# sv-goat/LLM-Inference-in-Distributed-Edge-Networks

Measured on AMD Instinct MI355X. Metric: WikiText-2 PPL + inter-stage bytes/token, Qwen2-0.5B 2-stage split; tokens/sec, higher is better.
Workload: dtype fp32; 1 GPU; model=qwen2-0.5b, global_batch=256, seq_len=512, stride=32, parallelism=local-pp2, codec=mixed_int4_int8, importance=regular_importance, transport=local, hip_graphs=True, gemm_precision=h3 split-fp16 (fp32-accurate), last_layer_rows=scored

## Files before the change

csrc/gemm.hip:

```cpp
#include <type_traits>
#include "common.h"
#include <algorithm>
#include <cstdlib>
#include <cstring>

enum { EPI_NONE = 0, EPI_BIAS = 1, EPI_RESID = 2, EPI_BIAS_RESID = 3, EPI_BIAS_GELU = 4, EPI_SWIGLU = 5,
       EPI_QKV_ROPE = 6, EPI_LSE = 7,
       EPI_F32 = 8, EPI_F32_BIAS = 9, EPI_F32_RESID = 10, EPI_F32_BIAS_RESID = 11, EPI_H3_BIAS_GELU = 12,
       EPI_H3_SWIGLU = 13, EPI_F32_QKV_ROPE = 14, EPI_F32_LSE = 15,
       EPI_F32_RESID_CS = 16,
       EPI_H3_LRP_SWIGLU = 17,
       EPI_F32_RESID_NP = 18 };
constexpr bool epi_f32(int e) { return e >= EPI_F32; }
constexpr bool epi_plain(int e) {
  return e == EPI_NONE || e == EPI_BIAS || e == EPI_RESID || e == EPI_BIAS_RESID || e == EPI_F32 ||
         e == EPI_F32_BIAS || e == EPI_F32_RESID || e == EPI_F32_BIAS_RESID || e == EPI_F32_RESID_CS ||
         e == EPI_F32_RESID_NP;
}

struct GemmArgs {
  const bf16_t* A; const bf16_t* B; bf16_t* C;
  int M, N, K, lda, ldb, ldc;
  const bf16_t* bias; const bf16_t* resid; int ldr;
  float* Cf; const float* biasf; const float* residf;
  float* qf; float* kf; float* vtf;
  float* vf;
  f16_t* planes; float* prinv; const float* bnd_a; const float* bnd_b; float bnd_c;
  float np_g, np_rn;
  bf16_t* qout; bf16_t* kout; bf16_t* vtout;
  const float* cosT; const float* sinT;
  int S, Hq, Hkv, s_pad; float q_scale;
  f16_t* kp; f16_t* vp; float kv_sk, kv_sv;
  const int64_t* targets; float* part_max; float* part_sum; float* tgt_logit; int nparts;
  const float* rscale; float* ssq_out;
  const float* colscale;
  const float* ssq_in; int ssq_parts; float norm_inv_k, norm_eps;
  int walk;
  int store_wait = 0;
  int h3k;
  int pairb;
  float alpha = 1.f;
  float out_scale = 1.f;
  float* raw = nullptr;
  bf16_t* rawb = nullptr;
};

__device__ __forceinline__ int a_kcol(const GemmArgs& a, int k) {
  if (a.pairb) return ((k >> 6) & 1 ? 0 : a.h3k) + ((k >> 7) << 6);
  return a.h3k ? h3_acol(k, a.h3k) : k;
}
__device__ __forceinline__ int b_kcol(const GemmArgs& a, int k) { return a.pairb ? (k >> 7) << 6 : k; }

template <bool F16>
__device__ __forceinline__ f32x4_t mfma16x32(bf16x8_t a, bf16x8_t b, f32x4_t c) {
  if constexpr (F16)
    return __builtin_amdgcn_mfma_f32_16x16x32_f16(__builtin_bit_cast(f16x8_t, a), __builtin_bit_cast(f16x8_t, b), c,
                                                  0, 0, 0);
  else
    return __builtin_amdgcn_mfma_f32_16x16x32_bf16(a, b, c, 0, 0, 0);
}

constexpr int BK = 64;
constexpr int GROUP_M = 8;

template <int BM_, int BN_, int NWM_, int NWN_>
struct Cfg {
  static constexpr int BM = BM_, BN = BN_, NWM = NWM_, NWN = NWN_;
  static constexpr int NW = NWM * NWN, NT = 64 * NW;
  static constexpr int WTM = BM / NWM, MI = WTM / 16;
  static_assert(BN / NWN == 64, "wave column slab must be 64");
  static constexpr int A_BYTES = BM * BK * 2, B_BYTES = BN * BK * 2, STAGE = A_BYTES + B_BYTES;
  static constexpr int A_INSTR = BM / 8 / NW, B_INSTR = BN / 8 / NW;
  static constexpr int LDS = 2 * STAGE;
};
using C128 = Cfg<128, 128, 2, 2>;

__device__ __forceinline__ int swz(int r) { return (r >> 1) & 7; }


__device__ __forceinline__ float gelu_erf(float x) { return 0.5f * x * (1.f + erff(x * 0.70710678118654752f)); }
__device__ __forceinline__ float silu(float x) { return fast_silu(x); }

template <int NI, int NW>
__device__ __forceinline__ void stage_ptrs(const bf16_t* __restrict__ src, int ld, int row0, int row_max, int wave,
                                           int lane, const bf16_t* (&p)[NI]) {
#pragma unroll
  for (int i = 0; i < NI; ++i) {
    const int blk = i * NW + wave;
    const int r = blk * 8 + (lane >> 3);
    const int c = (lane & 7) ^ swz(r);
    int gr = row0 + r;
    gr = gr < row_max ? gr : row_max - 1;
    p[i] = src + (size_t)gr * ld + c * 8;
  }
}
template <int NI, int NW>
__device__ __forceinline__ void stage_issue(const bf16_t* const (&p)[NI], int k0, char* lds, int wave) {
#pragma unroll
  for (int i = 0; i < NI; ++i) glds16(p[i] + k0, lds + (i * NW + wave) * 1024);
}

__device__ __forceinline__ bf16x8_t read_frag(const char* lds, int r, int c) {
  return *(const bf16x8_t*)(lds + r * 128 + ((c ^ swz(r)) << 4));
}

__device__ __forceinline__ void swiglu_h3_rowgroup(const GemmArgs& a, const f32x4_t (&acc4)[4], float f, u32x4_t& H,
                                                   u32x4_t& L) {
  const f32x2_t c1 = {-1.4426950408889634f * f, -1.4426950408889634f * f};
  const f32x2_t k2 = {f * f * a.out_scale, f * f * a.out_scale};
  u32x2_t hw[2], lw[2];
#pragma unroll
  for (int p = 0; p < 2; ++p) {
#pragma unroll
    for (int h = 0; h < 2; ++h) {
      const f32x2_t gg = {acc4[2 * p][2 * h], acc4[2 * p][2 * h + 1]};
      const f32x2_t uu = {acc4[2 * p + 1][2 * h], acc4[2 * p + 1][2 * h + 1]};
      f32x2_t o = gg * uu;
      const f32x2_t t = gg * c1;
      f32x2_t e = {__builtin_amdgcn_exp2f(t[0]), __builtin_amdgcn_exp2f(t[1])};
      e = e + f32x2_t{1.f, 1.f};
      o = o * f32x2_t{__builtin_amdgcn_rcpf(e[0]), __builtin_amdgcn_rcpf(e[1])};
      o = o * k2;
      const u32x2_t hl = split2h_pk(o[0], o[1]);
      hw[p][h] = hl[0];
// ... 750 lines not shown
                                            int lane, int wm, int wn) {
  const int g = lane >> 4;
  const int nw = n0 + wn * 112;
  const int P = a.N / 112;
  static_assert(!epi_f32(EPI), "fp32 epilogues of the 224-wide tiles: w4_f32_epilogue_224");
  constexpr bool RES = EPI == EPI_RESID || EPI == EPI_BIAS_RESID;
  u32x2_t rv[w7::MI][w7::NJ];
  float rsv[w7::MI];
#pragma unroll
  for (int i = 0; i < w7::MI; ++i) {
    int mr = m0 + wm * 64 + i * 16 + (lane & 15);
    mr = mr < a.M ? mr : a.M - 1;
    rsv[i] = a.rscale ? a.rscale[mr] : 1.f;
    if constexpr (RES) {
      const bf16_t* rrow = a.resid + (size_t)mr * a.ldr + nw + g * 4;
#pragma unroll
      for (int j = 0; j < w7::NJ; ++j) rv[i][j] = *(const u32x2_t*)(rrow + j * 16);
    }
  }
#pragma unroll
  for (int i = 0; i < w7::MI; ++i) {
    const int m = m0 + wm * 64 + i * 16 + (lane & 15);
    const bool ok = m < a.M;
    const float rs = rsv[i];
    float ss = 0.f;
    u32x2_t w[w7::NJ];
#pragma unroll
    for (int j = 0; j < w7::NJ; ++j) {
      const int n = nw + j * 16 + g * 4;
      float o[4] = {acc[i][j][0] * rs, acc[i][j][1] * rs, acc[i][j][2] * rs, acc[i][j][3] * rs};
      if constexpr (EPI == EPI_BIAS || EPI == EPI_BIAS_RESID) {
        const u32x2_t bw = *(const u32x2_t*)(a.bias + n);
        o[0] += bf_lo(bw[0]); o[1] += bf_hi(bw[0]); o[2] += bf_lo(bw[1]); o[3] += bf_hi(bw[1]);
      }
      if constexpr (RES) {
        const u32x2_t rw = rv[i][j];
        o[0] += bf_lo(rw[0]); o[1] += bf_hi(rw[0]); o[2] += bf_lo(rw[1]); o[3] += bf_hi(rw[1]);
      }
      w[j][0] = pack_bf2(o[0], o[1]);
      w[j][1] = pack_bf2(o[2], o[3]);
      const float v0 = bf_lo(w[j][0]), v1 = bf_hi(w[j][0]), v2 = bf_lo(w[j][1]), v3 = bf_hi(w[j][1]);
      ss += v0 * v0 + v1 * v1 + v2 * v2 + v3 * v3;
    }
    bf16_t* row = a.C + (size_t)(ok ? m : a.M - 1) * a.ldc + nw;
#pragma unroll
    for (int q2 = 0; q2 < 3; ++q2) {
      const u32x4_t wv = pair_swap16(w[2 * q2], w[2 * q2 + 1]);
      if (ok) *(u32x4_t*)(row + q2 * 32 + pair_col(g)) = wv;
    }
    if (ok) *(u32x2_t*)(row + 96 + g * 4) = w[6];
    if (a.ssq_out) {
      ss += __shfl_xor(ss, 16, 64);
      ss += __shfl_xor(ss, 32, 64);
      if (ok && g == 0) a.ssq_out[(size_t)m * P + nw / 112] = ss;
    }
  }
}

namespace w4 {
template <int BN> struct Geo {
  static constexpr int NJ = BN / 32;
  static constexpr int NB = BN / 32;
  static constexpr int BOFF = 32768, TB = 32768 + BN * 128;
  static constexpr int NR = 8 + NJ;
  static constexpr int MF = 8 * NJ;
  static constexpr int LDS = 2 * TB;
  static constexpr int LDS_R3 = 3 * 32768 + 2 * BN * 128;
};
template <int MF, int NR>
__device__ constexpr int slot_pos(int r) { return (r + 1) * MF / NR - 1; }
}

__device__ __forceinline__ int q192_feat(int col) {
  const int q = (col >> 4) & 3;
  return (col & ~63) | ((q == 1 ? 2 : q == 2 ? 1 : q) << 4) | (col & 15);
}

__device__ __forceinline__ void qkv192_bias(const GemmArgs& a, int n0, int lane, int wn, f32x4_t (&bw)[6]) {
  const int nw = n0 + wn * 96;
#pragma unroll
  for (int j = 0; j < 6; ++j) bw[j] = *(const f32x4_t*)(a.biasf + q192_feat(nw + j * 16) + (lane >> 4) * 4);
}

template <int RH>
__device__ __forceinline__ void qkv192_epilogue(const GemmArgs& a, f32x4_t (&c)[4][6], const f32x4_t (&bw)[6], int m0,
                                                int n0, int lane, int vw, int wn) {
  static_assert(RH == 0 || RH == 32, "192-wide QKV tiles: full rotary or none");
  const int g = lane >> 4;
  const int nw = n0 + wn * 96;
  int bi[4], pi[4];
  f32x4_t cs[4][2], sn[4][2];
#pragma unroll
  for (int i = 0; i < 4; ++i) {
    const int m = min(m0 + vw * 64 + i * 16 + (lane & 15), a.M - 1);
    bi[i] = m / a.S;
    pi[i] = m - bi[i] * a.S;
    if constexpr (RH == 32) {
#pragma unroll
      for (int hf = 0; hf < 2; ++hf) {
        cs[i][hf] = *(const f32x4_t*)(a.cosT + pi[i] * 32 + hf * 16 + g * 4);
        sn[i][hf] = *(const f32x4_t*)(a.sinT + pi[i] * 32 + hf * 16 + g * 4);
      }
    }
  }
#pragma unroll
  for (int i = 0; i < 4; ++i) {
    const int m = m0 + vw * 64 + i * 16 + (lane & 15);
    if (m >= a.M) continue;
    const int b = bi[i], pos = pi[i];
#pragma unroll
    for (int p = 0; p < 3; ++p) {
      const int col = nw + 32 * p;
      const int head = col >> 6;
      const int hf = ((col >> 4) & 3) ? 1 : 0;
      const int d = hf * 16 + g * 4;
      f32x4_t lo = c[i][2 * p] * a.alpha + bw[2 * p];
      f32x4_t hi = c[i][2 * p + 1] * a.alpha + bw[2 * p + 1];
      const bool is_v = head >= a.Hq + a.Hkv;
      if (!is_v) {
        if constexpr (RH == 32) {
          const f32x4_t cv = hf ? cs[i][1] : cs[i][0], sv = hf ? sn[i][1] : sn[i][0];
          const f32x4_t l2 = lo * cv - hi * sv;
          hi = hi * cv + lo * sv;
          lo = l2;
        }
        const float sc = head < a.Hq ? a.q_scale : 1.f;
        float* dst = head < a.Hq ? a.qf + (((size_t)b * a.Hq + head) * a.S + pos) * 64
                                 : a.kf + (((size_t)b * a.Hkv + (head - a.Hq)) * a.S + pos) * 64;
        if (head < a.Hq || a.kf) {
          *(f32x4_t*)(dst + d) = lo * sc;
          *(f32x4_t*)(dst + d + 32) = hi * sc;
        }
        if (head >= a.Hq && a.kp) {
          const float l4[4] = {lo[0], lo[1], lo[2], lo[3]}, h4[4] = {hi[0], hi[1], hi[2], hi[3]};
          store_k_planes4(a, b, head - a.Hq, pos, d, l4);
          store_k_planes4(a, b, head - a.Hq, pos, d + 32, h4);
        }
      } else {
        if (a.vf) {
          float* dst = a.vf + (((size_t)b * a.Hkv + (head - a.Hq - a.Hkv)) * a.S + pos) * 64;
          *(f32x4_t*)(dst + d) = lo;
          *(f32x4_t*)(dst + d + 32) = hi;
        }
        if (a.vtf) {
          float* dst = a.vtf + ((size_t)b * a.Hkv + (head - a.Hq - a.Hkv)) * 64 * (size_t)a.s_pad + pos;
#pragma unroll
          for (int r = 0; r < 4; ++r) {
            dst[(size_t)(d + r) * a.s_pad] = lo[r];
            dst[(size_t)(d + 32 + r) * a.s_pad] = hi[r];
          }
        }
        if (a.vp) {
#pragma unroll
          for (int r = 0; r < 4; ++r) {
            store_vt_plane1(a, b, head - a.Hq - a.Hkv, pos, d + r, lo[r]);
            store_vt_plane1(a, b, head - a.Hq - a.Hkv, pos, d + 32 + r, hi[r]);
          }
        }
      }
    }
  }
}

template <int RH>
__device__ __forceinline__ void qkv192_bf16_epilogue(const GemmArgs& a, f32x4_t (&c)[4][6], const float (&rq)[4],
                                                     int m0, int n0, int lane, int vw, int wn) {
  static_assert(RH == 0 || RH == 32, "192-wide QKV tiles: full rotary or none");
  const int g = lane >> 4;
  const int nw = n0 + wn * 96;
  u32x2_t bw[6];
#pragma unroll
  for (int j = 0; j < 6; ++j) bw[j] = *(const u32x2_t*)(a.bias + q192_feat(nw + j * 16) + g * 4);
  int bi[4], pi[4];
  f32x4_t cs[4][2], sn[4][2];
#pragma unroll
  for (int i = 0; i < 4; ++i) {
    const int m = min(m0 + vw * 64 + i * 16 + (lane & 15), a.M - 1);
    bi[i] = m / a.S;
    pi[i] = m - bi[i] * a.S;
    if constexpr (RH == 32) {
#pragma unroll
      for (int hf = 0; hf < 2; ++hf) {
        cs[i][hf] = *(const f32x4_t*)(a.cosT + pi[i] * 32 + hf * 16 + g * 4);
        sn[i][hf] = *(const f32x4_t*)(a.sinT + pi[i] * 32 + hf * 16 + g * 4);
      }
    }
  }
#pragma unroll
  for (int i = 0; i < 4; ++i) {
    const int m = m0 + vw * 64 + i * 16 + (lane & 15);
    if (m >= a.M) continue;
    const int b = bi[i], pos = pi[i];
#pragma unroll
    for (int p = 0; p < 3; ++p) {
      const int col = nw + 32 * p;
      const int head = col >> 6;
      const int hf = ((col >> 4) & 3) ? 1 : 0;
      const int d = hf * 16 + g * 4;
      const u32x2_t bl = bw[2 * p], bh = bw[2 * p + 1];
      f32x4_t lo = c[i][2 * p] * rq[i] + f32x4_t{bf_lo(bl[0]), bf_hi(bl[0]), bf_lo(bl[1]), bf_hi(bl[1])};
      f32x4_t hi = c[i][2 * p + 1] * rq[i] + f32x4_t{bf_lo(bh[0]), bf_hi(bh[0]), bf_lo(bh[1]), bf_hi(bh[1])};
      if (head < a.Hq + a.Hkv) {
        if constexpr (RH == 32) {
          const f32x4_t cv = hf ? cs[i][1] : cs[i][0], sv = hf ? sn[i][1] : sn[i][0];
          const f32x4_t l2 = lo * cv - hi * sv;
          hi = hi * cv + lo * sv;
          lo = l2;
        }
        const float sc = head < a.Hq ? a.q_scale : 1.f;
        bf16_t* dst = head < a.Hq ? a.qout + (((size_t)b * a.Hq + head) * a.S + pos) * 64
                                  : a.kout + (((size_t)b * a.Hkv + (head - a.Hq)) * a.S + pos) * 64;
        *(u32x2_t*)(dst + d) = u32x2_t{pack_bf2(lo[0] * sc, lo[1] * sc), pack_bf2(lo[2] * sc, lo[3] * sc)};
        *(u32x2_t*)(dst + d + 32) = u32x2_t{pack_bf2(hi[0] * sc, hi[1] * sc), pack_bf2(hi[2] * sc, hi[3] * sc)};
      } else {
        bf16_t* dst = a.vtout + ((size_t)b * a.Hkv + (head - a.Hq - a.Hkv)) * 64 * (size_t)a.s_pad + pos;
#pragma unroll
        for (int r = 0; r < 4; ++r) {
          dst[(size_t)(d + r) * a.s_pad] = f2bf(lo[r]);
          dst[(size_t)(d + 32 + r) * a.s_pad] = f2bf(hi[r]);
        }
      }
    }
  }
}

template <int EPI>
__device__ __forceinline__ void w4_f32_epilogue_224(const GemmArgs& a, f32x4_t (&acc)[8][7], int m0, int n0,
                                                    int lane, int wm, int wn) {
  constexpr bool NP = EPI == EPI_F32_RESID_NP;
  constexpr bool RESF = EPI == EPI_F32_RESID || EPI == EPI_F32_BIAS_RESID || EPI == EPI_F32_RESID_CS || NP;
  constexpr bool BIAS = EPI == EPI_F32_BIAS || EPI == EPI_F32_BIAS_RESID;
  constexpr bool CS = EPI == EPI_F32_RESID_CS;
  const int g = lane >> 4;
  const int nw = n0 + wn * 112;
  const int rbase = m0 + wm * 128 + (lane & 15);
  f32x4_t bw[BIAS || CS || NP ? 7 : 1];
  if constexpr (BIAS) {
#pragma unroll
    for (int j = 0; j < 7; ++j) bw[j] = *(const f32x4_t*)(a.biasf + nw + j * 16 + g * 4);
  }
  if constexpr (CS || NP) {
#pragma unroll
// ... 247 lines not shown
      }
    }
  };
  load_rs(m0);
  auto ktile = [&](int t, auto dmab_c, auto end_c) {
    const uint32_t bo = aslot(t), bn = aslot(t + 1);
    const uint32_t boB = PB ? ((t >> 1) & 1) * BSTRIDE : bo, bnB = PB ? (((t + 1) >> 1) & 1) * BSTRIDE : bn;
    __builtin_amdgcn_sched_barrier(0);
    using DM0 = std::integral_constant<int, R3 ? 2 : (SP2 && decltype(dmab_c)::value) ? 4 : 0>;
    if (kt == 0) mma(XA, XB, YA, YB, bo, boB, 1, std::true_type{}, DM0{}, std::true_type{}, dmab_c);
    else mma(XA, XB, YA, YB, bo, boB, 1, std::false_type{}, DM0{}, std::true_type{}, dmab_c);
    __builtin_amdgcn_sched_barrier(0);
    if (t + 1 < total) {
      constexpr int N0 = R3 ? 8 : (SP2 && decltype(dmab_c)::value) ? NB : 0;
      constexpr int TS = epi_tail_stores<EPI, BN>();
      if constexpr (TS > 0 && RING == 0) {
        if (kt == 0 && epi_full) wait_vm_lgkm0<N0 + TS>();
        else wait_vm_lgkm0<N0>();
      } else {
        wait_vm_lgkm0<N0>();
      }
    } else {
      asm volatile("s_waitcnt lgkmcnt(0)" ::: "memory");
    }
    if constexpr ((BN == 256 || BN == 192) && (RING == 0 || (SP2 && !decltype(dmab_c)::value))) {
#pragma unroll
      for (int i = 0; i < 8; ++i) asm volatile("" : "+v"(rs[i]));
    }
    __builtin_amdgcn_s_barrier();
    __builtin_amdgcn_sched_barrier(0);
    mma(YA, YB, XA, XB, bn, bnB, 0, std::false_type{}, std::integral_constant<int, R3 ? 3 : SP2 ? 5 : 1>{},
        std::true_type{}, dmab_c);
    __builtin_amdgcn_sched_barrier(0);
    asm volatile("s_waitcnt lgkmcnt(0)" ::: "memory");
    ++kt;
    if (decltype(end_c)::value && kt == nk) {
      MFMA_DRAIN();
      __builtin_amdgcn_sched_barrier(0);
      if constexpr (BN == 256 && EPI == EPI_H3_SWIGLU) {
        swiglu_h3_lines_4w<8>(a, acc, rs, m0, n0, lane, wm, wn);
        __builtin_amdgcn_sched_barrier(0);
      } else if constexpr (BN == 256 && EPI == EPI_H3_LRP_SWIGLU) {
        lrp_swiglu_4w(a, acc, m0, n0, lane, wm, wn);
        __builtin_amdgcn_sched_barrier(0);
      } else if constexpr (BN == 256) {
#pragma unroll
        for (int qd = 0; qd < 4; ++qd) {
          const int ih = qd >> 1, h = qd & 1;
          f32x4_t c[4][4];
          float rq[4];
#pragma unroll
          for (int i = 0; i < 4; ++i) {
            rq[i] = rs[ih * 4 + i];
#pragma unroll
            for (int j = 0; j < 4; ++j) {
              c[i][j] = acc[ih * 4 + i][h * 4 + j];
              asm volatile("" : "+v"(c[i][j]));
            }
          }
          if (n0 + wn * 128 + h * 64 < a.N) gemm_epilogue<EPI, RH, CQ>(a, c, m0, n0, lane, wm * 2 + ih, wn * 2 + h, rq);
          __builtin_amdgcn_sched_barrier(0);
        }
      } else if constexpr (BN == 192) {
        f32x4_t bw[6];
        if constexpr (EPI != EPI_QKV_ROPE) qkv192_bias(a, n0, lane, wn, bw);
#pragma unroll
        for (int ih = 0; ih < 2; ++ih) {
          f32x4_t c[4][6];
#pragma unroll
          for (int i = 0; i < 4; ++i)
#pragma unroll
            for (int j = 0; j < 6; ++j) {
              c[i][j] = acc[ih * 4 + i][j];
              asm volatile("" : "+v"(c[i][j]));
            }
          if constexpr (EPI == EPI_QKV_ROPE) {
            const float rq[4] = {rs[ih * 4], rs[ih * 4 + 1], rs[ih * 4 + 2], rs[ih * 4 + 3]};
            qkv192_bf16_epilogue<RH>(a, c, rq, m0, n0, lane, wm * 2 + ih, wn);
          } else {
            qkv192_epilogue<RH>(a, c, bw, m0, n0, lane, wm * 2 + ih, wn);
          }
          __builtin_amdgcn_sched_barrier(0);
        }
      } else if constexpr (epi_f32(EPI)) {
        w4_f32_epilogue_224<EPI>(a, acc, m0, n0, lane, wm, wn);
        __builtin_amdgcn_sched_barrier(0);
      } else {
#pragma unroll
        for (int ih = 0; ih < 2; ++ih) {
          f32x4_t c[4][NJ];
#pragma unroll
          for (int i = 0; i < 4; ++i)
#pragma unroll
            for (int j = 0; j < NJ; ++j) {
              c[i][j] = acc[ih * 4 + i][j];
              asm volatile("" : "+v"(c[i][j]));
            }
          w7_epilogue<EPI>(a, c, m0, n0, lane, wm * 2 + ih, wn);
          __builtin_amdgcn_sched_barrier(0);
        }
      }
      epi_full = a.store_wait && m0 + 256 <= a.M && n0 + BN <= a.N;
      tile += G;
      kt = 0;
      if (tile < walk.end) {
        tile_origin(tile, a.M, a.N, 256, BN, m0, n0);
        load_rs(m0);
      }
#pragma unroll
      for (int i = 0; i < 8; ++i) DS_READ_B128(XA[i], abase[0] + bn, i * 2048);
#pragma unroll
      for (int j = 0; j < NJ; ++j) DS_READ_B128(XB[j], bbase[0] + bnB, j * 2048);
      asm volatile("s_waitcnt lgkmcnt(0)" ::: "memory");
      __builtin_amdgcn_sched_barrier(0);
    }
  };
#pragma unroll 1
  for (int t = 0; t < total; t += PB ? 2 : 1) {
    if constexpr (PB) {
      ktile(t, std::true_type{}, std::false_type{});
      ktile(t + 1, std::false_type{}, std::true_type{});
    } else {
      ktile(t, std::true_type{}, std::true_type{});
    }
  }
  asm volatile("s_waitcnt vmcnt(0)" ::: "memory");
}

static int g_tile_override = 0;

static int num_cus() {
  static int n = 0;
  if (!n) {
    int dev = 0;
    (void)hipGetDevice(&dev);
    if (hipDeviceGetAttribute(&n, hipDeviceAttributeMultiprocessorCount, dev) != hipSuccess || n <= 0) n = 256;
  }
  return n;
}

template <int EPI, int RH, class CF>
static int launch_cfg(const GemmArgs& a, hipStream_t st) {
  const int grid = ((a.M + CF::BM - 1) / CF::BM) * ((a.N + CF::BN - 1) / CF::BN);
  static bool attr = false;
  if (!attr) {
    (void)hipFuncSetAttribute((const void*)gemm_bf16_kernel<EPI, RH, CF>, hipFuncAttributeMaxDynamicSharedMemorySize,
                              CF::LDS);
    attr = true;
  }
  hipLaunchKernelGGL((gemm_bf16_kernel<EPI, RH, CF>), dim3(grid), dim3(CF::NT), CF::LDS, st, a);
  return (int)hipGetLastError();
}

static int g_walk_override = [] {
  const char* e = getenv("EDGE_GEMM_WALK");
  return (e && (e[0] == '0' || e[0] == '1')) ? e[0] - '0' : -1;
}();

static int g_store_wait = -1;
static int store_wait() {
  if (g_store_wait < 0) {
    const char* e = getenv("EDGE_GEMM_STORE_WAIT");
    g_store_wait = (e && e[0] && e[0] != '0') ? 1 : 0;
  }
  return g_store_wait;
}

template <int EPI, int RH, int BN, bool PB, int RING = 0>
static int launch_4w_pb(const GemmArgs& args, hipStream_t st, int walk) {
  GemmArgs a = args;
  a.walk = g_walk_override >= 0 ? g_walk_override : walk;
  a.store_wait = store_wait();
  const int tiles = ((a.M + 255) / 256) * ((a.N + BN - 1) / BN);
  const int grid = std::min(tiles, num_cus());
  constexpr int lds = RING == 1 ? w4::Geo<BN>::LDS_R3 : w4::Geo<BN>::LDS;
  static bool attr = false;
  if (!attr) {
    (void)hipFuncSetAttribute((const void*)gemm_4w_kernel<EPI, RH, BN, PB, RING>,
                              hipFuncAttributeMaxDynamicSharedMemorySize, lds);
    attr = true;
  }
  hipLaunchKernelGGL((gemm_4w_kernel<EPI, RH, BN, PB, RING>), dim3(grid), dim3(256), lds, st, a);
  return (int)hipGetLastError();
}

static int g_ring = -1;
static int ring_mode(int bn) {
  if (g_ring < 0) {
    const char* e = getenv("EDGE_GEMM_RING");
    g_ring = 22;
    if (e && strlen(e) == 3 && strspn(e, "012") == 3) g_ring = atoi(e);
  }
  return (bn == 192 ? g_ring / 100 : bn == 224 ? g_ring / 10 : g_ring) % 10;
}

template <int EPI, int RH, int BN = 256>
static int launch_4w(const GemmArgs& a, hipStream_t st, int walk = 0) {
  if constexpr (epi_f32(EPI)) {
    if (a.pairb) {
      const int r = ring_mode(BN);
      if (r == 1) return launch_4w_pb<EPI, RH, BN, true, 1>(a, st, walk);
      if (r == 2) return launch_4w_pb<EPI, RH, BN, true, 2>(a, st, walk);
      return launch_4w_pb<EPI, RH, BN, true>(a, st, walk);
    }
  }
  return launch_4w_pb<EPI, RH, BN, false>(a, st, walk);
}

static bool use_224(int M, int N, int K, int epi) {
  if (!epi_plain(epi)) return false;
  if (N % 224 || N % 256 == 0 || K < 2 * BK) return false;
  if (g_tile_override) return g_tile_override == 224;
  return (long long)((M + 255) / 256) * (N / 224) >= 256;
}

template <int EPI, int RH = 0>
static int launch(const GemmArgs& a, hipStream_t st) {
  if constexpr (epi_plain(EPI)) {
    if (use_224(a.M, a.N, a.K, EPI)) return launch_4w<EPI, 0, 224>(a, st);
  }
  if constexpr (EPI == EPI_QKV_ROPE || EPI == EPI_F32_QKV_ROPE) {
    const long long tiles = (long long)((a.M + 255) / 256) * ((a.N + 255) / 256);
    if constexpr (RH == 0 || RH == 32) {
      const long long t192 = (long long)((a.M + 255) / 256) * (a.N / 192);
      if (a.N % 192 == 0 && a.N % 256 &&
          (g_tile_override == 192 || (EPI == EPI_F32_QKV_ROPE && t192 >= 256 && !g_tile_override)))
        return launch_4w<EPI, RH, 192>(a, st, 1);
    }
    if (g_tile_override == 256 || (EPI == EPI_F32_QKV_ROPE && tiles >= 256 && !g_tile_override))
      return launch_4w<EPI, RH>(a, st, 1);
    return launch_cfg<EPI, RH, C128>(a, st);
  } else if constexpr (EPI == EPI_LSE || EPI == EPI_F32_LSE) {
    const bool big = a.N % 128 == 0 && (long long)((a.M + 255) / 256) * ((a.N + 255) / 256) >= 256;
    if (big && g_tile_override != 128) return launch_4w<EPI, RH>(a, st);
    return launch_cfg<EPI, RH, C128>(a, st);
  } else {
    const int tn = (a.N + 255) / 256;
    const bool fits = a.N % 256 == 0 || (a.N % 128 == 0 && tn >= 4 && EPI != EPI_SWIGLU && EPI != EPI_H3_SWIGLU);
    const bool big = fits && ((long long)((a.M + 255) / 256) * tn >= 256);
    const bool use256 = g_tile_override ? g_tile_override == 256 && fits : big;
    if (!use256) return launch_cfg<EPI, RH, C128>(a, st);
    return launch_4w<EPI, RH>(a, st);
  }
}

EDGE_API int edge_gemm_set_tile(int t) {
  g_tile_override = t;
  return 0;
}

EDGE_API int edge_gemm_set_ring(int code) {
  const bool ok = code >= 0 && code / 100 <= 2 && code / 10 % 10 <= 2 && code % 10 <= 2;
  g_ring = ok ? code : -1;
  return 0;
}

EDGE_API int edge_gemm_set_store_wait(int on) {
  g_store_wait = on;
  return 0;
}

EDGE_API int edge_gemm_ssq_parts(int M, int N, int K, int act, int has_bias, int has_resid) {
  if (act) return N / 64;
  const int epi = has_bias ? (has_resid ? EPI_BIAS_RESID : EPI_BIAS) : (has_resid ? EPI_RESID : EPI_NONE);
  return use_224(M, N, K, epi) ? N / 112 : N / 64;
}

static int check_shapes(const GemmArgs& a) {
  if (a.M <= 0) return -1;
  if (a.N % 128 || a.K % BK || a.N <= 0 || a.K <= 0) return (int)hipErrorInvalidValue;
  if (a.lda % 8 || a.ldb % 8) return (int)hipErrorInvalidValue;
  return 0;
}

EDGE_API int edge_gemm(const void* A, const void* B, void* C, int M, int N, int K, int lda, int ldb, int ldc,
                       const void* bias, const void* resid, int ldr, int act, const float* rscale, float* ssq_out,
                       hipStream_t st) {
  GemmArgs a{};
  a.rscale = rscale; a.ssq_out = ssq_out;
  if (ssq_out && (N % 64 || act == 2)) return (int)hipErrorInvalidValue;
  a.A = (const bf16_t*)A; a.B = (const bf16_t*)B; a.C = (bf16_t*)C;
  a.M = M; a.N = N; a.K = K; a.lda = lda; a.ldb = ldb; a.ldc = ldc;
  a.bias = (const bf16_t*)bias; a.resid = (const bf16_t*)resid; a.ldr = ldr;
  const int chk = check_shapes(a);
  if (chk) return chk < 0 ? 0 : chk;
  if (ldc % 8 || ((uintptr_t)C & 15) || (resid && ldr % 4)) return (int)hipErrorInvalidValue;
  if (act == 2) return bias || resid ? (int)hipErrorInvalidValue : launch<EPI_SWIGLU>(a, st);
  if (act == 1) return resid || !bias ? (int)hipErrorInvalidValue : launch<EPI_BIAS_GELU>(a, st);
  if (bias && resid) return launch<EPI_BIAS_RESID>(a, st);
  if (bias) return launch<EPI_BIAS>(a, st);
  if (resid) return launch<EPI_RESID>(a, st);
  return launch<EPI_NONE>(a, st);
}

EDGE_API int edge_gemm_swiglu_raw(const void* A, const void* B, void* C, void* raw, int M, int N, int K, int lda,
                                  int ldb, int ldc, const float* rscale, hipStream_t st) {
  GemmArgs a{};
  a.rscale = rscale;
  a.A = (const bf16_t*)A; a.B = (const bf16_t*)B; a.C = (bf16_t*)C;
  a.M = M; a.N = N; a.K = K; a.lda = lda; a.ldb = ldb; a.ldc = ldc;
  a.rawb = (bf16_t*)raw;
  const int chk = check_shapes(a);
  if (chk) return chk < 0 ? 0 : chk;
  if (!raw || ((uintptr_t)raw & 15) || ldc % 8 || ((uintptr_t)C & 15)) return (int)hipErrorInvalidValue;
  return launch<EPI_SWIGLU>(a, st);
}

EDGE_API int edge_gemm_qkv_rope(const void* X, const void* W, const void* bias, void* q, void* k, void* vt,
                                const float* cosT, const float* sinT, int M, int K, int S, int Hq, int Hkv,
                                int rot_dim, int s_pad, float q_scale, const float* rscale, const float* ssq_in,
                                int ssq_parts, float norm_eps, hipStream_t st) {
  GemmArgs a{};
  a.rscale = rscale;
  a.ssq_in = ssq_in; a.ssq_parts = ssq_parts; a.norm_inv_k = 1.f / (float)K; a.norm_eps = norm_eps;
  if (ssq_in && ssq_parts != 8 && ssq_parts != 14) return (int)hipErrorInvalidValue;
  if (ssq_in && ((uintptr_t)ssq_in & 15)) return (int)hipErrorInvalidValue;
  a.A = (const bf16_t*)X; a.B = (const bf16_t*)W;
  a.M = M; a.N = (Hq + 2 * Hkv) * 64; a.K = K; a.lda = K; a.ldb = K;
  a.bias = (const bf16_t*)bias;
  a.qout = (bf16_t*)q; a.kout = (bf16_t*)k; a.vtout = (bf16_t*)vt;
  a.cosT = cosT; a.sinT = sinT; a.S = S; a.Hq = Hq; a.Hkv = Hkv; a.s_pad = s_pad;
  a.q_scale = q_scale;
  if (!bias || M % S) return (int)hipErrorInvalidValue;
  const int chk = check_shapes(a);
  if (chk) return chk < 0 ? 0 : chk;
  switch (rot_dim) {
    case 0: return launch<EPI_QKV_ROPE, 0>(a, st);
    case 8: return launch<EPI_QKV_ROPE, 4>(a, st);
    case 16: return launch<EPI_QKV_ROPE, 8>(a, st);
    case 32: return launch<EPI_QKV_ROPE, 16>(a, st);
// ... 207 lines not shown
```

llm_inference_in_distributed_edge_networks_amd/ops/__init__.py:

```python
from __future__ import annotations


import math

import torch

from . import reference as ref
from ._native import call, lib, ptr, stream

IL_BLOCK = ref.IL_BLOCK
s_pad = ref.s_pad
rope_tables = ref.rope_tables
interleave_gate_up = ref.interleave_gate_up
deinterleave_gate_up = ref.deinterleave_gate_up

_ACT = {None: 0, "gelu": 1, "swiglu_il": 2}




def _gpu(t: torch.Tensor) -> bool:
    return t.is_cuda


# ... 34 lines not shown
        call("edge_embedding_f32", ptr(ids), ptr(table), ptr(out), T, H, V, stream())
        return out
    _check_bf16(table)
    call("edge_embedding", ptr(ids), ptr(table), ptr(out), T, H, V, stream())
    return out


def _out_f32_or_h3(R: int, H: int, h3: float, device) -> torch.Tensor:
    return torch.empty(R, 2 * H, dtype=torch.float16, device=device) if h3 else \
        torch.empty(R, H, dtype=torch.float32, device=device)


def rmsnorm(x: torch.Tensor, w: torch.Tensor, eps: float, rows: torch.Tensor | None = None,
            h3: float = 0.0, rstd_out: torch.Tensor | None = None) -> torch.Tensor:
    if not _gpu(x):
        xs = x if rows is None else x.index_select(0, rows.long())
        if rstd_out is not None:
            rstd_out.copy_(ref.row_rstd(xs, eps))
        y = ref.rmsnorm(xs, w, eps)
        return ref.h3_act(y, h3) if h3 else y
    R = x.shape[0] if rows is None else rows.numel()
    H = x.shape[1]
    rows32 = None if rows is None else rows.to(torch.int32).contiguous()
    if x.dtype == torch.float32:
        _check_f32(x, w, rstd_out)
        y = _out_f32_or_h3(R, H, h3, x.device)
        if rstd_out is not None:
            assert rstd_out.shape == (R,)
            call("edge_rmsnorm_f32_rstd", ptr(x), ptr(w), ptr(y), ptr(rows32), R, H, float(eps), float(h3),
                 ptr(rstd_out), stream())
            return y
        call("edge_rmsnorm_f32", ptr(x), ptr(w), ptr(y), ptr(rows32), R, H, float(eps), float(h3), stream())
        return y
    if rstd_out is not None:
        raise TypeError("rstd_out: fp32 activations only")
    _check_bf16(x, w)
    y = torch.empty(R, H, dtype=x.dtype, device=x.device)
    call("edge_rmsnorm", ptr(x), ptr(w), ptr(y), ptr(rows32), R, H, float(eps), stream())
    return y


def layernorm(x, w, b, eps, rows=None, h3: float = 0.0):
    if not _gpu(x):
        y = ref.layernorm(x if rows is None else x.index_select(0, rows.long()), w, b, eps)
        return ref.h3_act(y, h3) if h3 else y
    R = x.shape[0] if rows is None else rows.numel()
    H = x.shape[1]
    rows32 = None if rows is None else rows.to(torch.int32).contiguous()
    if x.dtype == torch.float32:
        _check_f32(x, w, b)
        y = _out_f32_or_h3(R, H, h3, x.device)
        call("edge_layernorm_f32", ptr(x), ptr(w), ptr(b), None, None, ptr(y), None, ptr(rows32), R, H, float(eps),
             float(h3), 0.0, stream())
        return y
    _check_bf16(x, w, b)
    y = torch.empty(R, H, dtype=x.dtype, device=x.device)
    call("edge_layernorm", ptr(x), ptr(w), ptr(b), None, None, ptr(y), None, ptr(rows32), R, H, float(eps), stream())
    return y


def layernorm_dual(x, w1, b1, w2, b2, eps, h3: tuple[float, float] = (0.0, 0.0)):
    s1, s2 = h3
    if not _gpu(x):
        y1, y2 = ref.layernorm_dual(x, w1, b1, w2, b2, eps)
        return (ref.h3_act(y1, s1), ref.h3_act(y2, s2)) if s1 else (y1, y2)
    if x.dtype == torch.float32:
        _check_f32(x, w1, b1, w2, b2)
        R, H = x.shape
        y1, y2 = _out_f32_or_h3(R, H, s1, x.device), _out_f32_or_h3(R, H, s2, x.device)
        call("edge_layernorm_f32", ptr(x), ptr(w1), ptr(b1), ptr(w2), ptr(b2), ptr(y1), ptr(y2), None, R, H,
             float(eps), float(s1), float(s2), stream())
        return y1, y2
    _check_bf16(x, w1, b1, w2, b2)
    R, H = x.shape
    y1 = torch.empty_like(x)
    y2 = torch.empty_like(x)
    call("edge_layernorm", ptr(x), ptr(w1), ptr(b1), ptr(w2), ptr(b2), ptr(y1), ptr(y2), None, R, H, float(eps),
         stream())
    return y1, y2


def set_gemm_tile(tile: int) -> None:
    call("edge_gemm_set_tile", int(tile))


def set_gemm_ring(code: int) -> None:
    call("edge_gemm_set_ring", int(code))


def set_gemm_store_wait(on: int) -> None:
    call("edge_gemm_set_store_wait", int(on))


def gemm_ssq_parts(M: int, N: int, K: int, act=None, bias=False, residual=False) -> int:
    return int(lib().edge_gemm_ssq_parts(M, N, K, _ACT[act], int(bool(bias)), int(bool(residual))))


def row_ssq(x: torch.Tensor) -> torch.Tensor:
    if not _gpu(x):
        return ref.row_ssq(x)
    _check_bf16(x)
    T, H = x.shape
    out = torch.empty(T, H // 64, dtype=torch.float32, device=x.device)
    call("edge_row_ssq", ptr(x), ptr(out), T, H, stream())
    return out


def row_rscale(ssq: torch.Tensor, K: int, eps: float) -> torch.Tensor:
    if not ssq.is_cuda:
        return ref.rownorm_scale(ssq, K, eps)
    T, P = ssq.shape
    out = torch.empty(T, dtype=torch.float32, device=ssq.device)
    call("edge_row_rscale", ptr(ssq), ptr(out), T, P, K, float(eps), stream())
    return out


def _norm_scale(norm, K):
    ssq, eps = norm
    return row_rscale(ssq, K, eps)


def linear(x: torch.Tensor, w: torch.Tensor, bias=None, residual=None, act=None, out=None, norm=None,
           want_ssq: bool = False) -> torch.Tensor:
    if not _gpu(x):
        y = ref.linear(x, w, None, None, None, out_dtype=torch.float32) if norm is not None else None
        if norm is not None:
            ssq, eps = norm
            y = y * ref.rownorm_scale(ssq, x.shape[1], eps).view(-1, 1)
            if bias is not None:
                y = y + bias.float()
            if act == "swiglu_il":
                g, u = ref.deinterleave_gate_up(y)
                y = torch.nn.functional.silu(g) * u
            elif act == "gelu":
                y = ref.gelu(y)
            if residual is not None:
                y = y + residual.float()
            y = y.to(x.dtype)
        else:
            y = ref.linear(x, w, bias, residual, act)
        if out is not None:
            out.copy_(y)
            y = out
        if want_ssq:
            y._edge_ssq = ref.row_ssq(y)
        return y
    _check_bf16(x, w, bias, residual)
    M, K = x.shape
    N = w.shape[0]
    No = N // 2 if act == "swiglu_il" else N
    if out is None:
        out = torch.empty(M, No, dtype=x.dtype, device=x.device)
    rs = None if norm is None else _norm_scale(norm, K)
    ssq_out = torch.empty(M, gemm_ssq_parts(M, N, K, act, bias is not None, residual is not None),
                          dtype=torch.float32, device=x.device) if want_ssq else None
    call("edge_gemm", ptr(x), ptr(w), ptr(out), M, N, K, x.stride(0), w.stride(0), out.stride(0), ptr(bias),
         ptr(residual), 0 if residual is None else residual.stride(0), _ACT[act], ptr(rs), ptr(ssq_out), stream())
    if want_ssq:
        out._edge_ssq = ssq_out
    return out


def qkv_rope(x, wqkv, bqkv, cos, sin, B, S, Hq, Hkv, D, rot_dim, q_scale, norm=None):
    if not _gpu(x):
        if norm is not None:
            xs = (x.float() * ref.rownorm_scale(norm[0], x.shape[1], norm[1]).view(-1, 1))
# ... 588 lines not shown
```

llm_inference_in_distributed_edge_networks_amd/ops/_native.py:

```python
from __future__ import annotations

import ctypes
import os

import torch

from ..utils import poison as _poison

_HERE = os.path.dirname(os.path.abspath(__file__))
LIB_PATH = os.environ.get("EDGE_KERNEL_LIB") or os.path.join(os.path.dirname(_HERE), "_native", "libedge_kernels.so")

_lib = None

c_p = ctypes.c_void_p
c_i = ctypes.c_int
c_f = ctypes.c_float
c_ll = ctypes.c_longlong

_SIGS = {
    "edge_rmsnorm": [c_p, c_p, c_p, c_p, c_i, c_i, c_f, c_p],
    "edge_layernorm": [c_p, c_p, c_p, c_p, c_p, c_p, c_p, c_p, c_i, c_i, c_f, c_p],
    "edge_embedding": [c_p, c_p, c_p, c_i, c_i, c_i, c_p],
    "edge_gemm": [c_p, c_p, c_p, c_i, c_i, c_i, c_i, c_i, c_i, c_p, c_p, c_i, c_i, c_p, c_p, c_p],
    "edge_row_ssq": [c_p, c_p, c_i, c_i, c_p],
    "edge_row_rscale": [c_p, c_p, c_i, c_i, c_i, c_f, c_p],
    "edge_gemm_set_tile": [c_i],
    "edge_gemm_set_ring": [c_i],
    "edge_gemm_set_store_wait": [c_i],
    "edge_gemm_ssq_parts": [c_i, c_i, c_i, c_i, c_i, c_i],
    "edge_gemm_qkv_rope": [c_p, c_p, c_p, c_p, c_p, c_p, c_p, c_p, c_i, c_i, c_i, c_i, c_i, c_i, c_i, c_f, c_p, c_p,
                           c_i, c_f, c_p],
    "edge_gemm_lse": [c_p, c_p, c_p, c_p, c_p, c_p, c_i, c_i, c_i, c_i, c_f, c_p],
    "edge_lse_reduce": [c_p, c_p, c_p, c_p, c_i, c_i, c_p],
    "edge_flash_attn_fwd": [c_p, c_p, c_p, c_p, c_p, c_p, c_i, c_i, c_i, c_i, c_i, c_p],
    "edge_attn_lastrow": [c_p, c_p, c_p, c_i, c_i, c_i, c_i, c_p],
    "edge_attn_colsum": [c_p, c_p, c_p, c_p, c_i, c_i, c_i, c_i, c_p],
    "edge_head_combine": [c_p, c_p, c_p, c_i, c_i, c_i, c_f, c_f, c_p],
    "edge_select": [c_p, c_i, c_i, c_i, c_p, c_ll, c_i, c_f, c_ll, c_p],
    "edge_set_mask": [c_p, c_ll, c_i, c_i, c_i, c_p],
    "edge_channel_stats": [c_p, c_p, c_ll, c_p, c_i, c_i, c_i, c_i, c_i, c_i, c_p],
    "edge_rowmax": [c_p, c_p, c_i, c_i, c_p],
    "edge_pack": [c_p, c_p, c_ll, c_ll, c_ll, c_ll, c_ll, c_ll, c_i, c_i, c_i, c_i, c_i, c_i, c_i, c_i, c_i, c_i, c_i,
                  c_i, c_p],
    "edge_lrp_attn_bwd": [c_p, c_p, c_p, c_p, c_p, c_p, c_p, c_p, c_p, c_p, c_p, c_i, c_i, c_i, c_i, c_p],
    "edge_lrp_rope_pack": [c_p, c_p, c_p, c_p, c_p, c_p, c_i, c_i, c_i, c_i, c_i, c_f, c_p],
    "edge_swiglu_il": [c_p, c_p, c_ll, c_i, c_p],
    "edge_lrp_swiglu_bwd": [c_p, c_p, c_p, c_ll, c_i, c_p],
    "edge_lrp_gelu_bwd": [c_p, c_p, c_ll, c_p],
    "edge_lrp_ln_bwd": [c_p, c_p, c_p, c_p, c_p, c_p, c_p, c_p, c_i, c_i, c_p],
    "edge_ln_rstd": [c_p, c_p, c_i, c_i, c_f, c_p],
    "edge_unpack": [c_p, c_p, c_ll, c_ll, c_ll, c_ll, c_ll, c_ll, c_i, c_i, c_i, c_i, c_i, c_i, c_i, c_i, c_i, c_i,
                    c_i, c_i, c_p],
    "edge_rmsnorm_f32_rstd": [c_p, c_p, c_p, c_p, c_i, c_i, c_f, c_f, c_p, c_p],
    "edge_gemm_swiglu_raw": [c_p, c_p, c_p, c_p, c_i, c_i, c_i, c_i, c_i, c_i, c_p, c_p],
    "edge_gemm_f32_swiglu_raw": [c_p, c_p, c_p, c_p, c_i, c_i, c_i, c_i, c_i, c_i, c_i, c_p, c_f, c_f, c_p],
    "edge_gemm_f32_cs": [c_p, c_p, c_p, c_i, c_i, c_i, c_i, c_i, c_i, c_i, c_p, c_p, c_i, c_p, c_f,
                         c_p, c_p, c_p, c_p, c_f, c_p],
    "edge_lrp_attn_bwd_h3": [c_p] * 12 + [c_i] * 5 + [c_f] * 3 + [c_p],
    "edge_gemm_f32_lrp_swiglu": [c_p, c_p, c_p, c_p, c_i, c_i, c_i, c_i, c_i, c_i, c_i, c_f, c_p],
    "edge_gemm_f32_np_ok": [c_i, c_i, c_i],
    "edge_gemm_f32_np": [c_p, c_p, c_p, c_i, c_i, c_i, c_i, c_i, c_i, c_i, c_p, c_i, c_f, c_p, c_p, c_f, c_f, c_p, c_p,
                         c_p, c_p],
    "edge_row_rscale_mul": [c_p, c_p, c_p, c_i, c_i, c_i, c_f, c_p],
    "edge_gemm_f32": [c_p, c_p, c_p, c_i, c_i, c_i, c_i, c_i, c_i, c_i, c_p, c_p, c_i, c_i, c_p, c_f, c_f, c_p],
    "edge_gemm_qkv_rope_f32": [c_p, c_p, c_p, c_p, c_p, c_p, c_p, c_p, c_i, c_i, c_i, c_i, c_i, c_i, c_i, c_i, c_f,
                               c_f, c_p, c_p, c_f, c_f, c_p, c_p],
    "edge_flash_attn_fwd_h3p": [c_p, c_p, c_p, c_p, c_p, c_p, c_i, c_i, c_i, c_i, c_i, c_f, c_f, c_f, c_f, c_p, c_p],
    "edge_flash_attn_fwd_f32": [c_p, c_p, c_p, c_p, c_p, c_p, c_i, c_i, c_i, c_i, c_i, c_f, c_f, c_f, c_f, c_p],
    "edge_attn_lastrow_f32": [c_p, c_p, c_p, c_i, c_i, c_i, c_i, c_f, c_f, c_p],
    "edge_attn_colsum_f32": [c_p, c_p, c_p, c_p, c_i, c_i, c_i, c_i, c_f, c_f, c_p],
    "edge_rmsnorm_f32": [c_p, c_p, c_p, c_p, c_i, c_i, c_f, c_f, c_p],
    "edge_layernorm_f32": [c_p, c_p, c_p, c_p, c_p, c_p, c_p, c_p, c_i, c_i, c_f, c_f, c_f, c_p],
    "edge_split_h3": [c_p, c_p, c_p, c_i, c_i, c_f, c_p],
    "edge_embedding_f32": [c_p, c_p, c_p, c_i, c_i, c_i, c_p],
    "edge_lrp_rope_pack_h3": [c_p, c_p, c_p, c_p, c_p, c_p, c_p, c_p, c_i, c_i, c_i, c_i, c_i, c_f, c_p],
    "edge_lrp_rope_pack_h3_gs": [c_p, c_p, c_p, c_p, c_p, c_p, c_p, c_p, c_i, c_i, c_i, c_i, c_i, c_f, c_p],
    "edge_split_h3_dyn": [c_p, c_p, c_p, c_p, c_i, c_i, c_p],
    "edge_lrp_swiglu_bwd_h3": [c_p, c_p, c_p, c_p, c_p, c_i, c_i, c_p],
    "edge_lrp_gelu_bwd_h3": [c_p, c_p, c_p, c_p, c_i, c_i, c_p],
    "edge_act_h3": [c_p, c_p, c_ll, c_i, c_i, c_f, c_p],
    "edge_row_rstd_f32": [c_p, c_p, c_i, c_i, c_f, c_i, c_p],
    "edge_lrp_ln_bwd_f32": [c_p, c_p, c_p, c_p, c_p, c_p, c_p, c_i, c_i, c_p],
    "edge_group_absprod": [c_p, c_p, c_p, c_p, c_i, c_i, c_i, c_i, c_p],
    "edge_group_quant_err": [c_p, c_p, c_p, c_p, c_i, c_i, c_i, c_i, c_p],
    "edge_group_quant_err_chunks": [c_i],
    "edge_poison_lds": [c_p],
    "edge_poison_lds_bytes": [],
}


_LL_RESULT = {"edge_gemm_ws_floats"}


class NativeLibraryMissing(RuntimeError):
    pass


def tuning() -> bool:
    return os.environ.get("EDGE_TUNING", "0") not in ("", "0")


def available() -> bool:
    return os.path.exists(LIB_PATH)


def lib():
    global _lib
    if _lib is None:
        if not os.path.exists(LIB_PATH):
            raise NativeLibraryMissing(
                f"{LIB_PATH} not found: build the gfx950 kernels first "
                "(python -c 'import __graft_entry__ as g; g.build()')")
        L = ctypes.CDLL(LIB_PATH)
        for name, argt in _SIGS.items():
            if os.environ.get("EDGE_KERNEL_LIB") and not hasattr(L, name):
                continue
            fn = getattr(L, name)
            fn.argtypes = argt
            fn.restype = c_ll if name in _LL_RESULT else c_i
        _lib = L
    return _lib


def stream() -> int:
    return torch.cuda.current_stream().cuda_stream


def ptr(t) -> int | None:
    return None if t is None else t.data_ptr()


_NO_LAUNCH = {"edge_gemm_set_tile", "edge_gemm_set_ring", "edge_gemm_set_store_wait", "edge_gemm_ssq_parts", "edge_poison_lds", "edge_poison_lds_bytes",
              "edge_gemm_f32_np_ok", "edge_group_quant_err_chunks"}


def call(name: str, *args) -> None:
    if _poison.level() >= 2 and name not in _NO_LAUNCH:
        rc = lib().edge_poison_lds(stream())
        if rc != 0:
            raise RuntimeError(f"edge_poison_lds failed with HIP error {rc}")
    rc = getattr(lib(), name)(*args)
    if rc != 0:
        raise RuntimeError(f"{name} failed with HIP error {rc}")
```

Measured before the change: 765,800 tokens/s.

## Stage V^T fp16 planes through LDS for coalesced line stores in QKV epilogue

Moves the V transpose-plane stores out of the per-element QKV epilogue into a separate pass. For full 64-row aligned tiles, that pass writes the split fp16 values into a per-wave LDS scratch area, transposes them, and stores 16-byte contiguous lines along the sequence dimension instead of scattered 2-byte writes. This targets uncoalesced global stores of V^T. In exchange it adds extra LDS per block, which can lower occupancy, plus LDS round-trip work, and it keeps a fallback path for partial tiles.

```diff
diff --git a/csrc/gemm.hip b/csrc/gemm.hip
--- a/csrc/gemm.hip
+++ b/csrc/gemm.hip
@@ -40,6 +40,7 @@
   int h3k;
   int pairb;
   float alpha = 1.f;
+  int qkv_lines = 0;
   float out_scale = 1.f;
   float* raw = nullptr;
   bf16_t* rawb = nullptr;
@@ -956,6 +957,55 @@
   for (int j = 0; j < 6; ++j) bw[j] = *(const f32x4_t*)(a.biasf + q192_feat(nw + j * 16) + (lane >> 4) * 4);
 }
 
+constexpr int QKV_SCR_WAVE = 12288, QKV_SCR = 4 * QKV_SCR_WAVE, QKV_VT_RS = 144;
+static_assert(2 * 32 * QKV_VT_RS <= QKV_SCR_WAVE, "V^T staging fits the wave's slice");
+#define DS_WRITE_B32(vaddr, data, off) \
+  asm volatile("ds_write_b32 %0, %1 offset:%2" ::"v"(vaddr), "v"(data), "i"(off) : "memory")
+
+__device__ __forceinline__ bool qkv192_half_lines(const GemmArgs& a, int mb, int pos0) {
+  return a.qkv_lines && a.vp && mb + 64 <= a.M && !(pos0 & 63) && pos0 + 64 <= a.S;
+}
+
+__device__ __forceinline__ void qkv192_vt_lines(const GemmArgs& a, const f32x4_t (&c0)[4], const f32x4_t (&c1)[4],
+                                                const f32x4_t& b0, const f32x4_t& b1, int hv, int hf, int b, int pos0,
+                                                int lane, uint32_t scr) {
+  constexpr int RS = QKV_VT_RS;
+  const uint32_t wa = scr + (lane >> 4) * 4 * RS + (lane & 15) * 4;
+#pragma unroll
+  for (int ip = 0; ip < 2; ++ip) {
+#pragma unroll
+    for (int h = 0; h < 2; ++h) {
+      const f32x4_t e = (h ? c1[2 * ip] : c0[2 * ip]) * a.alpha + (h ? b1 : b0);
+      const f32x4_t o = (h ? c1[2 * ip + 1] : c0[2 * ip + 1]) * a.alpha + (h ? b1 : b0);
+#pragma unroll
+      for (int r = 0; r < 4; ++r) {
+        const u32x2_t t = split2h_pk(e[r] * a.kv_sv, o[r] * a.kv_sv);
+        DS_WRITE_B32(wa, t[0], (h * 16 + r) * RS + ip * 64);
+        DS_WRITE_B32(wa, t[1], (32 + h * 16 + r) * RS + ip * 64);
+      }
+    }
+  }
+  const uint32_t ra = scr + (lane >> 3) * RS + (lane & 7) * 16;
+  u32x4_t u[8];
+#pragma unroll
+  for (int k = 0; k < 8; ++k) DS_READ_B128(u[k], ra, k * 8 * RS);
+  asm volatile("s_waitcnt lgkmcnt(0)"
+               : "+v"(u[0]), "+v"(u[1]), "+v"(u[2]), "+v"(u[3]), "+v"(u[4]), "+v"(u[5]), "+v"(u[6]), "+v"(u[7])
+               :
+               : "memory");
+  f16_t* dst = a.vp + ((size_t)(b * a.Hkv + hv) * 2 * 64 + hf * 16 + (lane >> 3)) * a.s_pad + pos0 + (lane & 7) * 8;
+#pragma unroll
+  for (int k = 0; k < 8; ++k) {
+    const int d = ((k & 3) >> 1) * 32 + (k & 1) * 8;
+    u32x4_t w;
+    w[0] = __builtin_amdgcn_perm(u[k][1], u[k][0], 0x05040100u);
+    w[1] = __builtin_amdgcn_perm(u[k][3], u[k][2], 0x05040100u);
+    w[2] = __builtin_amdgcn_perm(u[k][1], u[k][0], 0x07060302u);
+    w[3] = __builtin_amdgcn_perm(u[k][3], u[k][2], 0x07060302u);
+    *(u32x4_t*)(dst + (size_t)((k >> 2) * 64 + d) * a.s_pad) = w;
+  }
+}
+
 template <int RH>
 __device__ __forceinline__ void qkv192_epilogue(const GemmArgs& a, f32x4_t (&c)[4][6], const f32x4_t (&bw)[6], int m0,
                                                 int n0, int lane, int vw, int wn) {
@@ -1024,14 +1074,55 @@
             dst[(size_t)(d + 32 + r) * a.s_pad] = hi[r];
           }
         }
-        if (a.vp) {
+      }
+    }
+  }
+}
+
+__device__ __forceinline__ void qkv192_vt_pass(const GemmArgs& a, const f32x4_t (&acc)[8][6], const f32x4_t (&bw)[6],
+                                               int m0, int n0, int lane, int wave, uint32_t scr0) {
+  const int wm = wave >> 1, wn = wave & 1;
+  const int nw = n0 + wn * 96;
+  if (!a.vp || (nw + 95) >> 6 < a.Hq + a.Hkv) return;
+  asm volatile("" : "+v"(lane), "+s"(wave));
+  const uint32_t scr = scr0 + wave * QKV_SCR_WAVE;
+#pragma unroll
+  for (int ih = 0; ih < 2; ++ih) {
+    const int mb = m0 + (wm * 2 + ih) * 64;
+    int mv = mb;
+    asm volatile("" : "+v"(mv));
+    const int b0 = __builtin_amdgcn_readfirstlane(mv / a.S);
+    const int pos0 = mb - b0 * a.S;
+    const bool lines = qkv192_half_lines(a, mb, pos0);
+#pragma unroll
+    for (int p = 0; p < 3; ++p) {
+      const int col = nw + 32 * p, head = col >> 6;
+      if (head < a.Hq + a.Hkv) continue;
+      const int hv = head - a.Hq - a.Hkv, hf = ((col >> 4) & 3) ? 1 : 0;
+      f32x4_t c0[4], c1[4];
+#pragma unroll
+      for (int i = 0; i < 4; ++i) {
+        c0[i] = acc[ih * 4 + i][2 * p];
+        c1[i] = acc[ih * 4 + i][2 * p + 1];
+        asm volatile("" : "+v"(c0[i]), "+v"(c1[i]));
+      }
+      if (lines) {
+        qkv192_vt_lines(a, c0, c1, bw[2 * p], bw[2 * p + 1], hv, hf, b0, pos0, lane, scr);
+      } else {
+#pragma unroll
+        for (int i = 0; i < 4; ++i) {
+          const int m = mb + i * 16 + (lane & 15);
+          if (m >= a.M) continue;
+          const int b = m / a.S, pos = m - b * a.S, d = hf * 16 + (lane >> 4) * 4;
+          const f32x4_t lo = c0[i] * a.alpha + bw[2 * p], hi = c1[i] * a.alpha + bw[2 * p + 1];
 #pragma unroll
           for (int r = 0; r < 4; ++r) {
-            store_vt_plane1(a, b, head - a.Hq - a.Hkv, pos, d + r, lo[r]);
-            store_vt_plane1(a, b, head - a.Hq - a.Hkv, pos, d + 32 + r, hi[r]);
+            store_vt_plane1(a, b, hv, pos, d + r, lo[r]);
+            store_vt_plane1(a, b, hv, pos, d + 32 + r, hi[r]);
           }
         }
       }
+      __builtin_amdgcn_sched_barrier(0);
     }
   }
 }
@@ -1445,6 +1536,10 @@
           }
           __builtin_amdgcn_sched_barrier(0);
         }
+        if constexpr (EPI == EPI_F32_QKV_ROPE) {
+          qkv192_vt_pass(a, acc, bw, m0, n0, lane, wave, lds_addr(smem) + 2 * TB);
+          __builtin_amdgcn_sched_barrier(0);
+        }
       } else if constexpr (epi_f32(EPI)) {
         w4_f32_epilogue_224<EPI>(a, acc, m0, n0, lane, wm, wn);
         __builtin_amdgcn_sched_barrier(0);
@@ -1491,6 +1586,7 @@
 }
 
 static int g_tile_override = 0;
+static int g_qkv_lines = 1;
 
 static int num_cus() {
   static int n = 0;
@@ -1536,7 +1632,10 @@
   a.store_wait = store_wait();
   const int tiles = ((a.M + 255) / 256) * ((a.N + BN - 1) / BN);
   const int grid = std::min(tiles, num_cus());
-  constexpr int lds = RING == 1 ? w4::Geo<BN>::LDS_R3 : w4::Geo<BN>::LDS;
+  constexpr bool scratch = BN == 192 && EPI == EPI_F32_QKV_ROPE && RING != 1;
+  constexpr int lds = (RING == 1 ? w4::Geo<BN>::LDS_R3 : w4::Geo<BN>::LDS) + (scratch ? QKV_SCR : 0);
+  static_assert(lds <= 160 * 1024, "LDS of a CU");
+  a.qkv_lines = scratch && g_qkv_lines;
   static bool attr = false;
   if (!attr) {
     (void)hipFuncSetAttribute((const void*)gemm_4w_kernel<EPI, RH, BN, PB, RING>,
@@ -1609,6 +1708,11 @@
 
 EDGE_API int edge_gemm_set_tile(int t) {
   g_tile_override = t;
+  return 0;
+}
+
+EDGE_API int edge_gemm_set_qkv_lines(int on) {
+  g_qkv_lines = on != 0;
   return 0;
 }
 
diff --git a/llm_inference_in_distributed_edge_networks_amd/ops/__init__.py b/llm_inference_in_distributed_edge_networks_amd/ops/__init__.py
--- a/llm_inference_in_distributed_edge_networks_amd/ops/__init__.py
+++ b/llm_inference_in_distributed_edge_networks_amd/ops/__init__.py
@@ -140,6 +140,10 @@
 
 def set_gemm_tile(tile: int) -> None:
     call("edge_gemm_set_tile", int(tile))
+
+
+def set_qkv_lines(on: bool) -> None:
+    call("edge_gemm_set_qkv_lines", int(bool(on)))
 
 
 def set_gemm_ring(code: int) -> None:
diff --git a/llm_inference_in_distributed_edge_networks_amd/ops/_native.py b/llm_inference_in_distributed_edge_networks_amd/ops/_native.py
--- a/llm_inference_in_distributed_edge_networks_amd/ops/_native.py
+++ b/llm_inference_in_distributed_edge_networks_amd/ops/_native.py
@@ -25,6 +25,7 @@
     "edge_row_ssq": [c_p, c_p, c_i, c_i, c_p],
     "edge_row_rscale": [c_p, c_p, c_i, c_i, c_i, c_f, c_p],
     "edge_gemm_set_tile": [c_i],
+    "edge_gemm_set_qkv_lines": [c_i],
     "edge_gemm_set_ring": [c_i],
     "edge_gemm_set_store_wait": [c_i],
     "edge_gemm_ssq_parts": [c_i, c_i, c_i, c_i, c_i, c_i],
@@ -130,7 +131,7 @@
     return None if t is None else t.data_ptr()
 
 
-_NO_LAUNCH = {"edge_gemm_set_tile", "edge_gemm_set_ring", "edge_gemm_set_store_wait", "edge_gemm_ssq_parts", "edge_poison_lds", "edge_poison_lds_bytes",
+_NO_LAUNCH = {"edge_gemm_set_tile", "edge_gemm_set_qkv_lines", "edge_gemm_set_ring", "edge_gemm_set_store_wait", "edge_gemm_ssq_parts", "edge_poison_lds", "edge_poison_lds_bytes",
               "edge_gemm_f32_np_ok", "edge_group_quant_err_chunks"}
 
 
```

Result: no change. 766,700 tokens/s, median of 5 (+0.1%).
